# mickeyjoe666/PHFPFAC

Measured on AMD Instinct MI355X. Metric: input GB/s scanned, higher is better.
Workload: dtype u8

## Files before the change

### phfpfac_amd/csrc/pfac_hip.hip

```cpp
#include <hip/hip_runtime.h>
#include <hip/hip_ext.h>

#include <stdint.h>
#include <stdio.h>
#include <stdlib.h>
#include <string.h>

#include <algorithm>
#include <chrono>
#include <mutex>
#include <type_traits>
#include <string>
#include <vector>

#include "pfac.h"
#include "pfac_fold.h"

namespace {

constexpr int WAVE = 64;
constexpr int SUB = WAVE * 16;
constexpr int SUBS = 4;
constexpr int WTILE = SUB * SUBS;
constexpr int MSUBS = 2;
// ... 1753 lines not shown
__global__ void __launch_bounds__(COUNT_THREADS_MAX)
pfac_count_kernel(const void *rec, const unsigned long long *tix, unsigned long long n_items, unsigned long long cap, unsigned n_states,
                  unsigned bins, unsigned long long *counts, unsigned long long *res) {
    extern __shared__ __attribute__((aligned(16))) unsigned char smem[];
    unsigned *lds = reinterpret_cast<unsigned *>(smem);
    const unsigned words = DIRECT ? n_states : 2 * bins;
    for (unsigned i = threadIdx.x; i < words; i += blockDim.x) lds[i] = 0;
    __syncthreads();
    const int lane = threadIdx.x & (WAVE - 1);
    const unsigned long long wstride = (unsigned long long)gridDim.x * (blockDim.x >> 6);
    unsigned long long counted = 0;
    unsigned phase = 0;
    bool peel = false;
    for (unsigned long long t = (unsigned long long)blockIdx.x * (blockDim.x >> 6) + (threadIdx.x >> 6); t < n_items; t += wstride) {
        if (BYTES == 0) {
            const unsigned long long i = t * WAVE + lane, n = cap;
            unsigned st = 0;
            bool have = i < n;
            if (have) st = static_cast<const pfac_record *>(rec)[i].state;
            have = have && st < n_states;
            counted += have;
            count_chunk<DIRECT>(lds, bins, counts, have, st, lane, phase, peel);
        } else {
            const unsigned long long e = tix[t], lo = e & TIX_BASE_MASK;
            const unsigned cnt = (unsigned)(e >> TIX_CNT_SHIFT);
            for (unsigned i0 = 0; i0 < cnt; i0 += WAVE) {
                const unsigned i = i0 + (unsigned)lane;
                unsigned pos, st = 0;
                bool have = i < cnt && lo + i < cap;
                if (have) heap_record<(BYTES ? BYTES : 4)>(rec, lo + i, t, pos, st);
                have = have && st < n_states;
                counted += have;
                count_chunk<DIRECT>(lds, bins, counts, have, st, lane, phase, peel);
            }
        }
    }
    __syncthreads();
    for (unsigned i = threadIdx.x; i < (DIRECT ? n_states : bins); i += blockDim.x) {
        const unsigned c = DIRECT ? lds[i] : lds[2 * i + 1];
        const unsigned st = DIRECT ? i : lds[2 * i] - 1u;
        if (c) __hip_atomic_fetch_add(counts + st, (unsigned long long)c, __ATOMIC_RELAXED, __HIP_MEMORY_SCOPE_AGENT);
    }
    counted = wave_sum64(counted);
    if (lane == 0 && counted) __hip_atomic_fetch_add(res, counted, __ATOMIC_RELAXED, __HIP_MEMORY_SCOPE_AGENT);
}

__global__ void pfac_sel_check_kernel(const pfac_record *sel, unsigned long long n, unsigned n_states, unsigned long long *bad) {
    const unsigned long long stride = (unsigned long long)gridDim.x * blockDim.x;
    bool wrong = false;
    for (unsigned long long i = (unsigned long long)blockIdx.x * blockDim.x + threadIdx.x; i < n; i += stride) {
        const pfac_record r = sel[i];
        wrong = wrong || r.state >= n_states || (i + 1 < n && sel[i + 1].pos <= r.pos);
    }
    if (wrong) bad[0] = 1ull;
}

constexpr int XGROUP = 64;
__global__ void pfac_tix_group_sum_kernel(const unsigned long long *tix, unsigned long long n_tiles, unsigned long long *gsum, unsigned n_groups) {
    const int lane = threadIdx.x & (WAVE - 1);
    const unsigned g = blockIdx.x * (blockDim.x >> 6) + (threadIdx.x >> 6);
    if (g >= n_groups) return;
    const unsigned long long t = (unsigned long long)g * XGROUP + lane;
    const unsigned c = t < n_tiles ? (unsigned)(tix[t] >> TIX_CNT_SHIFT) : 0u;
    const unsigned long long sum = wave_sum64(c);
    if (lane == 0) gsum[g] = sum;
}
__global__ void pfac_scan_groups_kernel(unsigned long long *gsum, unsigned n_groups) {
    __shared__ unsigned long long part[1024];
    const unsigned per = (n_groups + 1023u) / 1024u;
    const unsigned lo = threadIdx.x * per, hi = lo + per < n_groups ? lo + per : n_groups;
    unsigned long long sum = 0;
    for (unsigned i = lo; i < hi; i++) sum += gsum[i];
    part[threadIdx.x] = sum;
    __syncthreads();
    if (threadIdx.x == 0) {
        unsigned long long acc = 0;
        for (int i = 0; i < 1024; i++) { const unsigned long long v = part[i]; part[i] = acc; acc += v; }
    }
    __syncthreads();
    unsigned long long acc = part[threadIdx.x];
    for (unsigned i = lo; i < hi; i++) { const unsigned long long v = gsum[i]; gsum[i] = acc; acc += v; }
    if (hi == n_groups && lo < hi) gsum[n_groups] = acc;
}
template <int BYTES>
__global__ void pfac_expand_kernel(const void *rec, const unsigned long long *tix, unsigned long long n_tiles,
                                   const unsigned long long *gpre, unsigned n_groups, unsigned long long cap,
                                   unsigned long long first, unsigned long long n, pfac_record *out) {
    const int lane = threadIdx.x & (WAVE - 1);
    const unsigned g = blockIdx.x * (blockDim.x >> 6) + (threadIdx.x >> 6);
    if (g >= n_groups) return;
    const unsigned long long t = (unsigned long long)g * XGROUP + lane;
    const unsigned long long e = t < n_tiles ? tix[t] : 0ull;
    const unsigned c = (unsigned)(e >> TIX_CNT_SHIFT);
    const unsigned long long lo = e & TIX_BASE_MASK;
    const unsigned long long off = gpre[g] + (wave_incl_scan(c) - c);
    const unsigned long long end = first + n;
    for (int j = 0; j < XGROUP; j++) {
        const unsigned tc = __shfl(c, j, WAVE);
        if (tc == 0) continue;
        const unsigned long long tlo = __shfl(lo, j, WAVE), toff = __shfl(off, j, WAVE);
        if (toff >= end || toff + tc <= first) continue;
        for (unsigned i = (unsigned)lane; i < tc; i += WAVE) {
            const unsigned long long k = toff + i;
            if (k < first || k >= end || tlo + i >= cap) continue;
            pfac_record o;
            heap_record<BYTES>(rec, tlo + i, (unsigned long long)g * XGROUP + j, o.pos, o.state);
            out[k - first] = o;
        }
    }
}


__device__ __forceinline__ unsigned long long doc_lower_bound(const unsigned long long *off, unsigned long long n, unsigned long long x) {
    unsigned long long lo = 0, hi = n;
    while (lo < hi) {
        const unsigned long long mid = (lo + hi) >> 1;
        if (off[mid] < x) lo = mid + 1;
        else hi = mid;
    }
    return lo;
}
__device__ __forceinline__ unsigned long long doc_of(const unsigned long long *off, unsigned long long lo, unsigned long long hi, unsigned long long pos) {
    while (lo < hi) {
        const unsigned long long mid = (lo + hi + 1) >> 1;
        if (off[mid] <= pos) lo = mid;
        else hi = mid - 1;
    }
    return lo;
}
__device__ __forceinline__ void tile_docs(const unsigned long long *off, unsigned long long n_docs, unsigned long long t,
                                          unsigned long long n_tiles, unsigned long long &ds, unsigned long long &de,
                                          unsigned long long &dlo, unsigned long long &dhi) {
    ds = doc_lower_bound(off, n_docs + 1, t * WTILE);
    de = t + 1 == n_tiles ? n_docs + 1 : doc_lower_bound(off, n_docs + 1, (t + 1) * WTILE);
    const unsigned long long top = n_docs - 1;
    dlo = ds ? ds - 1 : 0;
    dhi = de ? de - 1 : 0;
    if (dlo > top) dlo = top;
    if (dhi > top) dhi = top;
    if (dhi < dlo) dhi = dlo;
}

struct DocWin {
    unsigned long long dlo, dhi, woff;
    unsigned n, top;
    bool win;
};
__device__ __forceinline__ DocWin doc_window(const unsigned long long *off, unsigned long long dlo, unsigned long long dhi, int lane) {
    DocWin w;
    w.dlo = dlo;
    w.dhi = dhi;
    w.win = dhi - dlo + 2 <= (unsigned long long)WAVE;
    w.n = w.win ? (unsigned)(dhi - dlo + 1) : 0u;
    w.top = w.n > 1 ? 1u << (31 - __clz(w.n - 1)) : 0u;
    w.woff = w.win && (unsigned)lane <= w.n ? off[dlo + lane] : ~0ull;
    return w;
}
__device__ __forceinline__ void doc_lookup(const DocWin &w, const unsigned long long *off, bool have, unsigned pos,
                                           unsigned long long &d, unsigned long long &base, unsigned long long &end) {
    if (w.win) {
        unsigned k = 0;
        for (unsigned step = w.top; step; step >>= 1) {
            const unsigned cand = k + step;
            const unsigned long long v = __shfl(w.woff, cand < w.n ? cand : 0u, WAVE);
            if (cand < w.n && v <= pos) k = cand;
        }
        d = w.dlo + k;
        base = __shfl(w.woff, k, WAVE);
        end = __shfl(w.woff, k + 1, WAVE);
    } else {
        d = have ? doc_of(off, w.dlo, w.dhi, pos) : w.dlo;
        base = have ? off[d] : 0ull;
        end = have ? off[d + 1] : 0ull;
    }
}
__device__ __forceinline__ int final_len(const short *flen, int freg, bool fsmall, bool have, unsigned st) {
    if (fsmall) return __shfl(freg, (int)st, WAVE);
    return have ? (int)flen[st] : 0;
}
#define GRID_THREAD ((unsigned long long)blockIdx.x * blockDim.x + threadIdx.x)
// ... 1098 lines not shown
        const unsigned l = rp_segment(so, cnt + 1, pos);
        const unsigned long long gs = so[l], ge = GAPS ? gs + sgl[l] : gs;
        unsigned long long pe;
        if (GAPS && pos < ge) {
            pe = min(ge, e);
            rp_merge(acc, in, (long long)(ssrc[l] + o - gs), n_avail, (unsigned)(pos - o), (unsigned)(pe - o));
        } else if constexpr (!TEMPLATES) {
            pe = min(so[l + 1], e);
            rp_merge(acc, rep, (long long)sro[l] + (long long)(o - ge), rep_size, (unsigned)(pos - o), (unsigned)(pe - o));
        } else {
            const unsigned long long m0 = ge + ssp[l], m1 = m0 + sml[l];
            if (pos < m0) {
                pe = min(m0, e);
                rp_merge(acc, rep, (long long)sro[l] + (long long)(o - ge), rep_size, (unsigned)(pos - o), (unsigned)(pe - o));
            } else if (pos < m1) {
                pe = min(m1, e);
                rp_merge(acc, in, (long long)(ssrc[l] + (ge - gs)) + (long long)(o - m0), n_avail, (unsigned)(pos - o), (unsigned)(pe - o));
            } else {
                pe = min(so[l + 1], e);
                rp_merge(acc, rep, (long long)sro[l] + (long long)ssp[l] + (long long)(o - m1), rep_size, (unsigned)(pos - o), (unsigned)(pe - o));
            }
        }
        return pe;
    });
}

template <bool TEMPLATES, bool GAPS>
__global__ void __launch_bounds__(4 * WAVE)
pfac_rp_doc_delta_kernel(const pfac_record *sel, unsigned long long n, const short *flen, const unsigned *roff,
                         const unsigned long long *X, const unsigned long long *gpre, unsigned long long *D,
                         const unsigned *split) {
    const int lane = threadIdx.x & (WAVE - 1);
    const unsigned long long b = (unsigned long long)blockIdx.x * 4 + (threadIdx.x >> 6), k = b * RP_BLOCK + (unsigned)lane;
    if (b * RP_BLOCK >= n) return;
    unsigned long long dk = 0;
    if (k < n) {
        const pfac_record r = sel[k];
        if constexpr (!TEMPLATES && GAPS) {
            dk = (unsigned long long)((long long)(roff[r.state + 1] - roff[r.state]) - (long long)flen[r.state]);
        } else {
            bool quote = false;
            if constexpr (TEMPLATES) quote = split[r.state] != PFAC_TEMPLATE_PLAIN;
            const long long R = (long long)(roff[r.state + 1] - roff[r.state]), L = (long long)flen[r.state];
            dk = (unsigned long long)(R + (quote ? L : 0ll) - (GAPS ? L : 0ll));
        }
    }
    unsigned long long base = 0;
    if (b > 0) {
        if constexpr (GAPS) {
            const pfac_record r = sel[b * RP_BLOCK - 1];
            base = X[b] + gpre[b / RP_GROUP] - ((unsigned long long)r.pos + (unsigned long long)flen[r.state]);
        } else {
            base = X[b] + gpre[b / RP_GROUP];
        }
    }
    rp_block_offsets(base, dk, k, n, D);
}

__global__ void pfac_rp_doc_offsets_kernel(const unsigned long long *off, const unsigned long long *doc_first,
                                           unsigned long long n_docs, const unsigned long long *D, unsigned long long n,
                                           unsigned long long *out_off) {
    const unsigned long long stride = (unsigned long long)gridDim.x * blockDim.x;
    for (unsigned long long d = (unsigned long long)blockIdx.x * blockDim.x + threadIdx.x; d <= n_docs; d += stride) {
        const unsigned long long f = doc_first[d];
        out_off[d] = off[d] + (n ? D[f < n ? f : n] : 0ull);
    }
}

__device__ __forceinline__ unsigned ndigits32(unsigned v) {
    return 1u + (v >= 10u) + (v >= 100u) + (v >= 1000u) + (v >= 10000u) + (v >= 100000u) + (v >= 1000000u) + (v >= 10000000u) +
           (v >= 100000000u) + (v >= 1000000000u);
}
__device__ __forceinline__ unsigned ndigits64(unsigned long long v) {
    return v < 1000000000ull ? ndigits32((unsigned)v) : 9u + ndigits32((unsigned)(v / 1000000000ull));
}
__device__ __forceinline__ unsigned text_line_len(unsigned long long pos, unsigned id) {
    const unsigned dp = ndigits64(pos);
    return 12u + (dp < 4u ? 4u : dp) + 16u + ndigits32(id) + 1u;
}
constexpr int TEXT_LINE_MAX = 12 + 18 + 16 + 10 + 1;
constexpr int TEXT_IMG = 16 + WAVE * TEXT_LINE_MAX + 15;

template <int BYTES>
__global__ void pfac_text_size_kernel(const void *rec, const unsigned long long *tix, unsigned long long n_tiles, unsigned long long cap,
                                      unsigned long long base, const int *idmap, unsigned long long *gsum, unsigned n_groups) {
    const int lane = threadIdx.x & (WAVE - 1);
    const unsigned g = blockIdx.x * (blockDim.x >> 6) + (threadIdx.x >> 6);
    if (g >= n_groups) return;
    const unsigned long long t = (unsigned long long)g * XGROUP + lane;
    const unsigned long long e = t < n_tiles ? tix[t] : 0ull;
    const unsigned c = (unsigned)(e >> TIX_CNT_SHIFT);
    const unsigned long long lo = e & TIX_BASE_MASK;
    unsigned long long total = 0;
    for (int j = 0; j < XGROUP; j++) {
        const unsigned tc = __shfl(c, j, WAVE);
        if (tc == 0) continue;
        const unsigned long long tlo = __shfl(lo, j, WAVE);
        unsigned long long sum = 0;
        for (unsigned i = (unsigned)lane; i < tc && tlo + i < cap; i += WAVE) {
            unsigned pos, st;
            heap_record<BYTES>(rec, tlo + i, (unsigned long long)g * XGROUP + j, pos, st);
            sum += text_line_len(base + pos, (unsigned)idmap[st]);
        }
        total += sum;
    }
    total = wave_sum64(total);
    if (lane == 0) gsum[g] = total;
}

__device__ __forceinline__ void put_digits32(unsigned char *p, unsigned v, unsigned nd) {
    for (unsigned k = nd; k-- > 0;) { const unsigned q = v / 10u; p[k] = (unsigned char)('0' + (v - q * 10u)); v = q; }
}

template <int BYTES>
__global__ __launch_bounds__(256) void pfac_text_format_kernel(const void *rec, const unsigned long long *tix, unsigned long long n_tiles,
                                                               unsigned long long cap, unsigned long long base, const int *idmap,
                                                               const unsigned long long *gpre, unsigned n_groups, unsigned char *text) {
    __shared__ __attribute__((aligned(16))) unsigned char img_all[4][(TEXT_IMG + 15) / 16 * 16];
    const int lane = threadIdx.x & (WAVE - 1);
    unsigned char *img = img_all[threadIdx.x >> 6];
    const unsigned g = blockIdx.x * (blockDim.x >> 6) + (threadIdx.x >> 6);
    if (g >= n_groups) return;
    const unsigned long long t = (unsigned long long)g * XGROUP + lane;
    const unsigned long long e = t < n_tiles ? tix[t] : 0ull;
    const unsigned c = (unsigned)(e >> TIX_CNT_SHIFT);
    const unsigned long long lo = e & TIX_BASE_MASK;
    unsigned long long at = gpre[g];
    for (int j = 0; j < XGROUP; j++) {
        const unsigned tc = __shfl(c, j, WAVE);
        if (tc == 0) continue;
        const unsigned long long tlo = __shfl(lo, j, WAVE);
        for (unsigned c0 = 0; c0 < tc; c0 += WAVE) {
            const unsigned i = c0 + (unsigned)lane;
            const bool have = i < tc && tlo + i < cap;
            unsigned pos = 0, st = 0, id = 0, len = 0, dp = 0, di = 0;
            unsigned long long gp = 0;
            if (have) {
                heap_record<BYTES>(rec, tlo + i, (unsigned long long)g * XGROUP + j, pos, st);
                id = (unsigned)idmap[st];
                gp = base + pos;
                dp = ndigits64(gp);
                di = ndigits32(id);
                len = 12u + (dp < 4u ? 4u : dp) + 16u + di + 1u;
            }
            const unsigned incl = wave_incl_scan(len);
            const unsigned total = bcast_last(incl);
            const unsigned a0 = (unsigned)(at & 15ull);
            if (have) {
                unsigned char *p = img + a0 + (incl - len);
                const char *h = "At position ";
#pragma unroll
                for (int k = 0; k < 12; k++) p[k] = (unsigned char)h[k];
                p += 12;
                for (unsigned k = dp; k < 4u; k++) *p++ = ' ';
                if (gp < 1000000000ull) put_digits32(p, (unsigned)gp, dp);
                else {
                    const unsigned hi = (unsigned)(gp / 1000000000ull), lo9 = (unsigned)(gp - (unsigned long long)hi * 1000000000ull);
                    put_digits32(p, hi, dp - 9u);
                    put_digits32(p + (dp - 9u), lo9, 9u);
                }
                p += dp;
                const char *m = ", match pattern ";
#pragma unroll
                for (int k = 0; k < 16; k++) p[k] = (unsigned char)m[k];
                p += 16;
                put_digits32(p, id, di);
                p[di] = (unsigned char)'\n';
            }
            wave_lds_sync();
            unsigned char *dst = text + (at - a0);
            const unsigned end = a0 + total;
            const unsigned b_lo = a0 ? 16u : 0u, b_hi = end & ~15u;
            if (b_hi > b_lo) {
                for (unsigned o = b_lo + 16u * (unsigned)lane; o < b_hi; o += 16u * WAVE)
                    __builtin_nontemporal_store(*reinterpret_cast<const u32x4 *>(img + o), reinterpret_cast<u32x4 *>(dst + o));
                if (a0 && (unsigned)lane < 16u - a0) dst[a0 + lane] = img[a0 + lane];
                if ((unsigned)lane < end - b_hi) dst[b_hi + lane] = img[b_hi + lane];
            } else {
                if (a0 + (unsigned)lane < end) dst[a0 + lane] = img[a0 + lane];
            }
            wave_lds_sync();
            at += total;
        }
    }
}

__device__ __forceinline__ unsigned long long splitmix64(unsigned long long x) {
    x += 0x9E3779B97F4A7C15ull;
    x = (x ^ (x >> 30)) * 0xBF58476D1CE4E5B9ull;
    x = (x ^ (x >> 27)) * 0x94D049BB133111EBull;
    return x ^ (x >> 31);
}

__global__ void pfac_fill_random_kernel(unsigned long long *dst, unsigned long long n_words, unsigned long long seed) {
    const unsigned long long stride = (unsigned long long)gridDim.x * blockDim.x;
    for (unsigned long long i = (unsigned long long)blockIdx.x * blockDim.x + threadIdx.x; i < n_words; i += stride)
        dst[i] = splitmix64(seed + i);
}

__global__ void pfac_fill_tiled_kernel(unsigned char *dst, unsigned long long n, const unsigned char *pat,
                                       unsigned period, unsigned long long phase) {
    const unsigned long long stride = (unsigned long long)gridDim.x * blockDim.x * 16;
    for (unsigned long long i = ((unsigned long long)blockIdx.x * blockDim.x + threadIdx.x) * 16; i < n; i += stride) {
        unsigned k = (unsigned)((phase + i) % period);
        if (i + 16 <= n) {
            union { unsigned char b[16]; uint4 v; } u;
#pragma unroll
            for (int j = 0; j < 16; j++) { u.b[j] = pat[k]; k = k + 1 == period ? 0 : k + 1; }
            *reinterpret_cast<uint4 *>(dst + i) = u.v;
        } else {
            for (unsigned long long j = i; j < n; j++) { dst[j] = pat[k]; k = k + 1 == period ? 0 : k + 1; }
// ... 1710 lines not shown
    }
    if (n_tiles == 0) {
        if (ctx->event_timing) HIP_TRY(ctx, hipEventRecord(s.ev1, s.stream));
        __atomic_store_n(s.h_ctl + H_DONE, 1u, __ATOMIC_RELEASE);
    }
    return PFAC_OK;
}

int pfac_scan_finish(pfac_ctx *ctx, int slot, uint64_t *n_matches) {
    int rc = check_slot(ctx, slot);
    if (rc) return rc;
    Slot &s = ctx->slots[slot];
    if (!s.scanned) return fail(ctx, PFAC_E_STATE, "pfac_scan_finish without a scan");
    USE_DEVICE(ctx);
    rc = wait_scan(ctx, s);
    if (rc) return rc;
    if (s.last_tiles == 0 && s.h2d_issued) HIP_TRY(ctx, hipEventSynchronize(s.ev_h2d));
    s.pending = false;
    const uint64_t total = host_u64(s, H_MATCHES);
    s.last_total = total;
    s.last_used = host_u64(s, H_USED);
    if (n_matches) *n_matches = total;
#ifdef PFAC_TRACE_BUILD
    if (s.dbg.p && !ctx->plan.knobs.trace_file.empty()) {
        std::vector<unsigned long long> h(8 * 64 * 32);
        if (hipMemcpy(h.data(), s.dbg.p, h.size() * 8, hipMemcpyDeviceToHost) == hipSuccess) {
            if (FILE *f = fopen(ctx->plan.knobs.trace_file.c_str(), "wb")) { fwrite(h.data(), 8, h.size(), f); fclose(f); }
        }
    }
#endif
    if (s.h_ctl[2] != 0) {
        s.clean[0] = s.clean[1] = false;
        return fail(ctx, PFAC_E_INTERNAL, "scan kernel reported a timeout (flags " + std::to_string(s.h_ctl[2]) +
                                          ": 4 arrivals, 8 record base, 16 batch ring)");
    }
    if (ctx->plan.knobs.dense < 0 && ctx->plan.lay_d.stage_cap && s.last_tiles >= 64) {
        const uint64_t ovf = s.h_ctl[3];
        if (!ctx->dense && ovf * 4 > s.last_tiles) ctx->dense = true;
        else if (ctx->dense && ovf * 16 < s.last_tiles) ctx->dense = false;
    }
    if (ctx->plan.lag2_ok && ctx->plan.knobs.lag != 1 && ctx->plan.knobs.lag != 2 && s.last_tiles >= 64) {
        const uint64_t ovf2 = s.h_ctl[6];
        if (ctx->lag2 && ovf2 * 16 > s.last_tiles) ctx->lag2 = false;
        else if (!ctx->lag2 && ovf2 * 64 < s.last_tiles) ctx->lag2 = true;
    }
    if (s.last_used > s.last_cap)
        return fail(ctx, PFAC_E_OVERFLOW, "record array too small: " + std::to_string(total) + " matches need " +
                                              std::to_string(s.last_used) + " records of capacity (pfac_scan_capacity_hint)");
    return PFAC_OK;
}

int pfac_scan_elapsed_ms(pfac_ctx *ctx, int slot, float *ms) {
    int rc = check_slot(ctx, slot);
    if (rc) return rc;
    if (!ms) return fail(ctx, PFAC_E_ARG, "null argument");
    Slot &s = ctx->slots[slot];
    if (!s.scanned) return fail(ctx, PFAC_E_STATE, "no scan to time");
    USE_DEVICE(ctx);
    rc = wait_scan(ctx, s);
    if (rc) return rc;
    if (s.last_tiles == 0) *ms = 0.0f;
    else if (ctx->event_timing) {
        HIP_TRY(ctx, hipEventElapsedTime(ms, s.ev0, s.ev1));
        ctx->clk_diff_ms += *ms - (double)(host_u64(s, H_T1) - host_u64(s, H_T0)) * ctx->tick_ms;
        ctx->clk_n++;
    }
    else *ms = (float)((double)(host_u64(s, H_T1) - host_u64(s, H_T0)) * ctx->tick_ms);
    return PFAC_OK;
}

static int expand_records(pfac_ctx *ctx, Slot &s, const void *src, uint64_t first, uint64_t n, pfac_record *d_out) {
    if (s.pending) return fail(ctx, PFAC_E_STATE, "records requested before pfac_scan_finish");
    if (!in_window(first, n, s.last_total)) return fail(ctx, PFAC_E_ARG, "records [first, first + n) exceed the scan's match count");
    int rc = last_scan_usable(ctx, s, "", SCAN_FITS);
    if (rc) return rc;
    if (n == 0 || s.last_tiles == 0) return PFAC_OK;
    const unsigned n_groups = (unsigned)((s.last_tiles + XGROUP - 1) / XGROUP);
    rc = ensure_gsum(ctx, s, n_groups);
    if (rc) return rc;
    const unsigned gblocks = (n_groups + 3) / 4;
    hipLaunchKernelGGL(pfac_tix_group_sum_kernel, dim3(gblocks), dim3(256), 0, s.stream, s.tile_index.p,
                       (unsigned long long)s.last_tiles, s.gsum.p, n_groups);
    hipLaunchKernelGGL(pfac_scan_groups_kernel, dim3(1), dim3(1024), 0, s.stream, s.gsum.p, n_groups);
    auto ek = by_width(s.last_rec_bytes, [](auto w) { return pfac_expand_kernel<w()>; });
    hipLaunchKernelGGL(ek, dim3(gblocks), dim3(256), 0, s.stream, src, s.tile_index.p, (unsigned long long)s.last_tiles,
                       s.gsum.p, n_groups, (unsigned long long)s.last_cap, (unsigned long long)first, (unsigned long long)n, d_out);
    HIP_TRY(ctx, hipGetLastError());
    return PFAC_OK;
}

int pfac_scan_format(pfac_ctx *ctx, int slot, int *record_bytes, uint64_t *n_tiles, uint64_t *used) {
    int rc = check_slot(ctx, slot);
    if (rc) return rc;
    Slot &s = ctx->slots[slot];
    if (!s.scanned) return fail(ctx, PFAC_E_STATE, "no scan yet");
    if (record_bytes) *record_bytes = s.last_rec_bytes;
    if (n_tiles) *n_tiles = s.last_tiles;
    if (used) *used = s.last_used;
    return PFAC_OK;
}

int pfac_scan_capacity_hint(pfac_ctx *ctx, int slot, uint64_t *capacity) {
    int rc = check_slot(ctx, slot);
    if (rc) return rc;
    Slot &s = ctx->slots[slot];
    if (!s.scanned || !capacity) return fail(ctx, PFAC_E_STATE, "pfac_scan_capacity_hint: no finished scan");
    const uint64_t a = s.last_used + s.last_used / 8, b = s.last_total + s.last_total / 4;
    *capacity = (a > b ? a : b) + 65536;
    return PFAC_OK;
}

int pfac_records_expand(pfac_ctx *ctx, int slot, const void *d_records, uint64_t first, uint64_t n, pfac_record *d_out) {
    int rc = check_slot(ctx, slot);
    if (rc) return rc;
    Slot &s = ctx->slots[slot];
    const void *src = d_records ? d_records : s.records.p;
    if (!s.scanned) return fail(ctx, PFAC_E_STATE, "pfac_records_expand without a scan");
    if (!src || (!d_out && n) || ((uintptr_t)d_out & 7)) return fail(ctx, PFAC_E_ARG, "pfac_records_expand: bad buffer");
    USE_DEVICE(ctx);
    return expand_records(ctx, s, src, first, n, d_out);
}

int pfac_records_d2h(pfac_ctx *ctx, int slot, const void *d_records, pfac_record *host, uint64_t first, uint64_t n) {
    int rc = check_slot(ctx, slot);
    if (rc) return rc;
    Slot &s = ctx->slots[slot];
    const void *src = d_records ? d_records : s.records.p;
    if (n == 0) return PFAC_OK;
    if (!s.scanned) return fail(ctx, PFAC_E_STATE, "pfac_records_d2h without a scan");
    if (!src || !host) return fail(ctx, PFAC_E_ARG, "pfac_records_d2h: null buffer");
    USE_DEVICE(ctx);
    rc = s.wide.ensure(ctx, s.stream, n, n);
    if (rc) return rc;
    rc = expand_records(ctx, s, src, first, n, s.wide.p);
    if (rc) return rc;
    HIP_TRY(ctx, hipMemcpyAsync(host, s.wide.p, n * sizeof(pfac_record), hipMemcpyDeviceToHost, s.stream));
    return PFAC_OK;
}

int pfac_records_d2h_packed(pfac_ctx *ctx, int slot, const void *d_records, void *host_words, uint64_t n_words,
                            uint64_t *host_tile_index) {
    int rc = check_slot(ctx, slot);
    if (rc) return rc;
    Slot &s = ctx->slots[slot];
    const void *src = d_records ? d_records : s.records.p;
    if (!s.scanned || s.last_rec_bytes == 8) return fail(ctx, PFAC_E_STATE, "pfac_records_d2h_packed: the slot's last scan did not produce compact records");
    if (!src || (!host_words && n_words) || !host_tile_index) return fail(ctx, PFAC_E_ARG, "pfac_records_d2h_packed: null buffer");
    if (n_words > s.last_cap) return fail(ctx, PFAC_E_ARG, "pfac_records_d2h_packed: more words than the record array holds");
    USE_DEVICE(ctx);
    if (n_words) HIP_TRY(ctx, hipMemcpyAsync(host_words, src, n_words * (uint64_t)s.last_rec_bytes, hipMemcpyDeviceToHost, s.stream));
    if (s.last_tiles) HIP_TRY(ctx, hipMemcpyAsync(host_tile_index, s.tile_index.p, s.last_tiles * 8, hipMemcpyDeviceToHost, s.stream));
    return PFAC_OK;
}

int pfac_records_packed_device(pfac_ctx *ctx, int slot, const void *d_records, void *d_words_out, uint64_t n_words,
                               uint64_t *d_tile_index_out) {
    int rc = check_slot(ctx, slot);
    if (rc) return rc;
    Slot &s = ctx->slots[slot];
    const void *src = d_records ? d_records : s.records.p;
    if (!s.scanned || s.pending || s.last_rec_bytes == 8) return fail(ctx, PFAC_E_STATE, "pfac_records_packed_device: the slot's last finished scan did not produce compact records");
    rc = last_scan_usable(ctx, s, "", SCAN_FITS);
    if (rc) return rc;
    if (!d_tile_index_out || (d_words_out && !src)) return fail(ctx, PFAC_E_ARG, "pfac_records_packed_device: null buffer");
    if (n_words > s.last_cap) return fail(ctx, PFAC_E_ARG, "pfac_records_packed_device: more words than the record array holds");
    USE_DEVICE(ctx);
    if (d_words_out && n_words && d_words_out != src)
        HIP_TRY(ctx, hipMemcpyAsync(d_words_out, src, n_words * (uint64_t)s.last_rec_bytes, hipMemcpyDeviceToDevice, s.stream));
    if (s.last_tiles) HIP_TRY(ctx, hipMemcpyAsync(d_tile_index_out, s.tile_index.p, s.last_tiles * 8, hipMemcpyDeviceToDevice, s.stream));
    return PFAC_OK;
}

int pfac_emit_text_device(pfac_ctx *ctx, int slot, const void *d_records, uint64_t base, uint64_t *n_bytes) {
    int rc = check_slot(ctx, slot);
    if (rc) return rc;
    if (!n_bytes) return fail(ctx, PFAC_E_ARG, "null argument");
    *n_bytes = 0;
    if (!ctx->have_table) return fail(ctx, PFAC_E_STATE, "no table uploaded");
    Slot &s = ctx->slots[slot];
    const void *src = d_records ? d_records : s.records.p;
    rc = last_scan_usable(ctx, s, "pfac_emit_text_device", SCAN_FINISHED | SCAN_IDMAP | SCAN_FITS);
    if (rc) return rc;
    if (base + (1ull << 32) >= 1000000000000000000ull) return fail(ctx, PFAC_E_ARG, "pfac_emit_text_device: positions must stay below 10^18");
    s.text_bytes = 0;
    if (s.last_total == 0 || s.last_tiles == 0) return PFAC_OK;
    if (!src) return fail(ctx, PFAC_E_ARG, "null record buffer");
    USE_DEVICE(ctx);
    const unsigned n_groups = (unsigned)((s.last_tiles + XGROUP - 1) / XGROUP);
    rc = ensure_gsum(ctx, s, n_groups);
    if (rc) return rc;
    const unsigned gblocks = (n_groups + 3) / 4;
    auto sk = by_width(s.last_rec_bytes, [](auto w) { return pfac_text_size_kernel<w()>; });
    hipLaunchKernelGGL(sk, dim3(gblocks), dim3(256), 0, s.stream, src, s.tile_index.p, (unsigned long long)s.last_tiles,
                       (unsigned long long)s.last_cap, (unsigned long long)base, ctx->plan.d_idmap, s.gsum.p, n_groups);
    hipLaunchKernelGGL(pfac_scan_groups_kernel, dim3(1), dim3(1024), 0, s.stream, s.gsum.p, n_groups);
    HIP_TRY(ctx, hipGetLastError());
    unsigned long long total = 0;
    HIP_TRY(ctx, hipMemcpyAsync(&total, s.gsum.p + n_groups, 8, hipMemcpyDeviceToHost, s.stream));
    HIP_TRY(ctx, hipStreamSynchronize(s.stream));
    rc = s.text.ensure(ctx, s.stream, total + 32, total + total / 8 + 4096);
    if (rc) return rc;
    auto fk = by_width(s.last_rec_bytes, [](auto w) { return pfac_text_format_kernel<w()>; });
    hipLaunchKernelGGL(fk, dim3(gblocks), dim3(256), 0, s.stream, src, s.tile_index.p, (unsigned long long)s.last_tiles,
                       (unsigned long long)s.last_cap, (unsigned long long)base, ctx->plan.d_idmap, s.gsum.p, n_groups, s.text.p);
    HIP_TRY(ctx, hipGetLastError());
    s.text_bytes = total;
    *n_bytes = total;
    return PFAC_OK;
}

int pfac_text_d2h(pfac_ctx *ctx, int slot, void *host, uint64_t first, uint64_t n) {
    int rc = check_slot(ctx, slot);
    if (rc) return rc;
    Slot &s = ctx->slots[slot];
    if (!in_window(first, n, s.text_bytes)) return fail(ctx, PFAC_E_ARG, "pfac_text_d2h: range exceeds the text of the slot's last pfac_emit_text_device");
    if (n == 0) return PFAC_OK;
    if (!host) return fail(ctx, PFAC_E_ARG, "null buffer");
    USE_DEVICE(ctx);
    HIP_TRY(ctx, hipMemcpyAsync(host, s.text.p + first, n, hipMemcpyDeviceToHost, s.stream));
    return PFAC_OK;
}

void *pfac_slot_text(pfac_ctx *ctx, int slot) { return check_slot(ctx, slot) ? nullptr : ctx->slots[slot].text.p; }

int pfac_slot_sync(pfac_ctx *ctx, int slot) {
    int rc = check_slot(ctx, slot);
    if (rc) return rc;
    USE_DEVICE(ctx);
    HIP_TRY(ctx, hipStreamSynchronize(ctx->slots[slot].stream));
    if (ctx->slots[slot].h2d_issued) HIP_TRY(ctx, hipEventSynchronize(ctx->slots[slot].ev_h2d));
    return PFAC_OK;
}

int pfac_records_checksum(pfac_ctx *ctx, int slot, const void *d_records, uint64_t n, uint64_t base, uint64_t *checksum) {
    int rc = check_slot(ctx, slot);
    if (rc) return rc;
    if (!checksum) return fail(ctx, PFAC_E_ARG, "null argument");
    if (!ctx->have_table) return fail(ctx, PFAC_E_STATE, "no table uploaded");
    Slot &s = ctx->slots[slot];
    const void *src = d_records ? d_records : s.records.p;
    rc = n ? last_scan_usable(ctx, s, "pfac_records_checksum", SCAN_FINISHED | SCAN_IDMAP | SCAN_FITS) : PFAC_OK;
    if (rc) return rc;
    if (!src && n) return fail(ctx, PFAC_E_ARG, "null record buffer");
    USE_DEVICE(ctx);
    HIP_TRY(ctx, hipMemsetAsync(s.sum.p, 0, 16, s.stream));
    if (n && s.last_tiles) {
        auto ck = by_width(s.last_rec_bytes, [](auto w) { return pfac_checksum_kernel<w()>; });
        hipLaunchKernelGGL(ck, dim3(1024), dim3(256), 0, s.stream, src, s.tile_index.p, (unsigned long long)s.last_tiles,
                           (unsigned long long)s.last_cap, (unsigned long long)base, ctx->plan.d_idmap, s.sum.p);
        HIP_TRY(ctx, hipGetLastError());
    }
    HIP_TRY(ctx, hipMemcpyAsync(s.h_ctl + H_CHECKSUM, s.sum.p, 8, hipMemcpyDeviceToHost, s.stream));
    HIP_TRY(ctx, hipStreamSynchronize(s.stream));
    *checksum = host_u64(s, H_CHECKSUM);
    return PFAC_OK;
}

}

namespace {

using CountKernel = void (*)(const void *, const unsigned long long *, unsigned long long, unsigned long long, unsigned, unsigned,
                             unsigned long long *, unsigned long long *);

int count_run(pfac_ctx *ctx, Slot &s, const std::string &fn, const void *heap, bool is_sel, const pfac_record *sel, uint64_t n_sel,
              bool check_sel, uint64_t *d_counts, uint64_t n_states, uint32_t flags, uint64_t *n_counted) {
    if (flags > PFAC_COUNT_ACCUMULATE) return fail(ctx, PFAC_E_ARG, fn + ": flags must be 0 or PFAC_COUNT_ACCUMULATE");
    if (n_states != (uint64_t)ctx->plan.base.num_final)
        return fail(ctx, PFAC_E_ARG, fn + ": n_states must be num_final of the uploaded table (" + std::to_string(ctx->plan.base.num_final) + ")");
    if ((uintptr_t)d_counts & 7) return fail(ctx, PFAC_E_ARG, fn + ": d_counts must be 8-byte aligned");
    const bool own = d_counts == nullptr, acc = (flags & PFAC_COUNT_ACCUMULATE) != 0;
    if (own && acc && s.cnt.done && s.cnt_table != ctx->table_gen)
        return fail(ctx, PFAC_E_STATE, fn + ": the slot's counts belong to an earlier table; they cannot be added to");
    const uint64_t expect = is_sel ? n_sel : s.last_total;
    const uint64_t n_items = is_sel ? (n_sel + WAVE - 1) / WAVE : s.last_tiles;
    if (!(is_sel ? (const void *)sel : heap) && n_items) return fail(ctx, PFAC_E_ARG, "null record buffer");
    USE_DEVICE(ctx);
    int rc = ensure_gsum(ctx, s, 1);
    if (rc) return rc;
    unsigned long long *res = s.gsum.p;
    const unsigned ns = (unsigned)n_states;
    if (check_sel && n_sel) {
        HIP_TRY(ctx, hipMemsetAsync(res, 0, 16, s.stream));
        const unsigned blocks = (unsigned)std::min<uint64_t>((n_sel + 255) / 256, 1024);
        hipLaunchKernelGGL(pfac_sel_check_kernel, dim3(blocks), dim3(256), 0, s.stream, sel, (unsigned long long)n_sel, ns, res + 1);
        rc = pass_words(ctx, s, res + 1, 1, H_PASS1);
        if (rc) return rc;
// ... 1516 lines not shown
```

Baseline: 5335.

## Split each 64-tile group across several waves in expand and text kernels

The expand, text-size and text-format kernels now give each wave a unit of XUNIT tiles instead of a whole 64-tile group, multiplying the number of waves by XGROUP/XUNIT. The text-size kernel runs one block per group and writes per-unit byte offsets, so the format kernel can start each unit at the right text position. This targets poor parallelism and load imbalance when few groups exist or when match counts are skewed. In exchange each wave still loads the group's tile index and prefix-scans it, so that work is repeated, and an extra offset array is kept in the gsum buffer. Launch bounds and restrict qualifiers are also added.

```diff
diff --git a/phfpfac_amd/csrc/pfac_hip.hip b/phfpfac_amd/csrc/pfac_hip.hip
--- a/phfpfac_amd/csrc/pfac_hip.hip
+++ b/phfpfac_amd/csrc/pfac_hip.hip
@@ -1859,20 +1859,30 @@
     for (unsigned i = lo; i < hi; i++) { const unsigned long long v = gsum[i]; gsum[i] = acc; acc += v; }
     if (hi == n_groups && lo < hi) gsum[n_groups] = acc;
 }
+#ifndef PFAC_XUNIT
+#define PFAC_XUNIT 8
+#endif
+constexpr int XUNIT = PFAC_XUNIT;
+constexpr int XUNITS = XGROUP / XUNIT;
+static_assert(XUNIT >= 4 && XUNIT <= XGROUP && (XUNIT & (XUNIT - 1)) == 0, "PFAC_XUNIT: 4, 8, 16, 32 or 64");
+
 template <int BYTES>
-__global__ void pfac_expand_kernel(const void *rec, const unsigned long long *tix, unsigned long long n_tiles,
-                                   const unsigned long long *gpre, unsigned n_groups, unsigned long long cap,
-                                   unsigned long long first, unsigned long long n, pfac_record *out) {
+__global__ void __launch_bounds__(256, 8)
+pfac_expand_kernel(const void *__restrict__ rec, const unsigned long long *__restrict__ tix, unsigned long long n_tiles,
+                   const unsigned long long *__restrict__ gpre, unsigned n_units, unsigned long long cap,
+                   unsigned long long first, unsigned long long n, pfac_record *__restrict__ out) {
     const int lane = threadIdx.x & (WAVE - 1);
-    const unsigned g = blockIdx.x * (blockDim.x >> 6) + (threadIdx.x >> 6);
-    if (g >= n_groups) return;
+    const unsigned u = blockIdx.x * (blockDim.x >> 6) + (threadIdx.x >> 6);
+    if (u >= n_units) return;
+    const unsigned g = u / XUNITS;
+    const int j0 = (int)(u % XUNITS) * XUNIT;
     const unsigned long long t = (unsigned long long)g * XGROUP + lane;
     const unsigned long long e = t < n_tiles ? tix[t] : 0ull;
     const unsigned c = (unsigned)(e >> TIX_CNT_SHIFT);
     const unsigned long long lo = e & TIX_BASE_MASK;
     const unsigned long long off = gpre[g] + (wave_incl_scan(c) - c);
     const unsigned long long end = first + n;
-    for (int j = 0; j < XGROUP; j++) {
+    for (int j = j0; j < j0 + XUNIT; j++) {
         const unsigned tc = __shfl(c, j, WAVE);
         if (tc == 0) continue;
         const unsigned long long tlo = __shfl(lo, j, WAVE), toff = __shfl(off, j, WAVE);
@@ -3137,17 +3147,19 @@
 constexpr int TEXT_IMG = 16 + WAVE * TEXT_LINE_MAX + 15;
 
 template <int BYTES>
-__global__ void pfac_text_size_kernel(const void *rec, const unsigned long long *tix, unsigned long long n_tiles, unsigned long long cap,
-                                      unsigned long long base, const int *idmap, unsigned long long *gsum, unsigned n_groups) {
-    const int lane = threadIdx.x & (WAVE - 1);
-    const unsigned g = blockIdx.x * (blockDim.x >> 6) + (threadIdx.x >> 6);
-    if (g >= n_groups) return;
+__global__ void __launch_bounds__(XUNITS * WAVE, 8)
+pfac_text_size_kernel(const void *__restrict__ rec, const unsigned long long *__restrict__ tix, unsigned long long n_tiles,
+                      unsigned long long cap, unsigned long long base, const int *__restrict__ idmap,
+                      unsigned long long *__restrict__ gsum, unsigned long long *__restrict__ uoff) {
+    __shared__ unsigned long long unit_bytes[XUNITS];
+    const int lane = threadIdx.x & (WAVE - 1), w = threadIdx.x >> 6;
+    const unsigned g = blockIdx.x;
     const unsigned long long t = (unsigned long long)g * XGROUP + lane;
     const unsigned long long e = t < n_tiles ? tix[t] : 0ull;
     const unsigned c = (unsigned)(e >> TIX_CNT_SHIFT);
     const unsigned long long lo = e & TIX_BASE_MASK;
     unsigned long long total = 0;
-    for (int j = 0; j < XGROUP; j++) {
+    for (int j = w * XUNIT; j < (w + 1) * XUNIT; j++) {
         const unsigned tc = __shfl(c, j, WAVE);
         if (tc == 0) continue;
         const unsigned long long tlo = __shfl(lo, j, WAVE);
@@ -3160,7 +3172,14 @@
         total += sum;
     }
     total = wave_sum64(total);
-    if (lane == 0) gsum[g] = total;
+    if (lane == 0) unit_bytes[w] = total;
+    __syncthreads();
+    if (threadIdx.x < XUNITS) {
+        unsigned long long front = 0;
+        for (int k = 0; k < (int)threadIdx.x; k++) front += unit_bytes[k];
+        uoff[(unsigned long long)g * XUNITS + threadIdx.x] = front;
+        if (threadIdx.x == XUNITS - 1) gsum[g] = front + unit_bytes[XUNITS - 1];
+    }
 }
 
 __device__ __forceinline__ void put_digits32(unsigned char *p, unsigned v, unsigned nd) {
@@ -3168,20 +3187,24 @@
 }
 
 template <int BYTES>
-__global__ __launch_bounds__(256) void pfac_text_format_kernel(const void *rec, const unsigned long long *tix, unsigned long long n_tiles,
-                                                               unsigned long long cap, unsigned long long base, const int *idmap,
-                                                               const unsigned long long *gpre, unsigned n_groups, unsigned char *text) {
+__global__ void __launch_bounds__(256, 8)
+pfac_text_format_kernel(const void *__restrict__ rec, const unsigned long long *__restrict__ tix, unsigned long long n_tiles,
+                        unsigned long long cap, unsigned long long base, const int *__restrict__ idmap,
+                        const unsigned long long *__restrict__ gpre, const unsigned long long *__restrict__ uoff, unsigned n_units,
+                        unsigned char *__restrict__ text) {
     __shared__ __attribute__((aligned(16))) unsigned char img_all[4][(TEXT_IMG + 15) / 16 * 16];
     const int lane = threadIdx.x & (WAVE - 1);
     unsigned char *img = img_all[threadIdx.x >> 6];
-    const unsigned g = blockIdx.x * (blockDim.x >> 6) + (threadIdx.x >> 6);
-    if (g >= n_groups) return;
+    const unsigned u = blockIdx.x * (blockDim.x >> 6) + (threadIdx.x >> 6);
+    if (u >= n_units) return;
+    const unsigned g = u / XUNITS;
+    const int j0 = (int)(u % XUNITS) * XUNIT;
     const unsigned long long t = (unsigned long long)g * XGROUP + lane;
     const unsigned long long e = t < n_tiles ? tix[t] : 0ull;
     const unsigned c = (unsigned)(e >> TIX_CNT_SHIFT);
     const unsigned long long lo = e & TIX_BASE_MASK;
-    unsigned long long at = gpre[g];
-    for (int j = 0; j < XGROUP; j++) {
+    unsigned long long at = gpre[g] + uoff[u];
+    for (int j = j0; j < j0 + XUNIT; j++) {
         const unsigned tc = __shfl(c, j, WAVE);
         if (tc == 0) continue;
         const unsigned long long tlo = __shfl(lo, j, WAVE);
@@ -5058,9 +5081,10 @@
     hipLaunchKernelGGL(pfac_tix_group_sum_kernel, dim3(gblocks), dim3(256), 0, s.stream, s.tile_index.p,
                        (unsigned long long)s.last_tiles, s.gsum.p, n_groups);
     hipLaunchKernelGGL(pfac_scan_groups_kernel, dim3(1), dim3(1024), 0, s.stream, s.gsum.p, n_groups);
+    const unsigned n_units = n_groups * XUNITS;
     auto ek = by_width(s.last_rec_bytes, [](auto w) { return pfac_expand_kernel<w()>; });
-    hipLaunchKernelGGL(ek, dim3(gblocks), dim3(256), 0, s.stream, src, s.tile_index.p, (unsigned long long)s.last_tiles,
-                       s.gsum.p, n_groups, (unsigned long long)s.last_cap, (unsigned long long)first, (unsigned long long)n, d_out);
+    hipLaunchKernelGGL(ek, dim3((n_units + 3) / 4), dim3(256), 0, s.stream, src, s.tile_index.p, (unsigned long long)s.last_tiles,
+                       s.gsum.p, n_units, (unsigned long long)s.last_cap, (unsigned long long)first, (unsigned long long)n, d_out);
     HIP_TRY(ctx, hipGetLastError());
     return PFAC_OK;
 }
@@ -5163,12 +5187,13 @@
     if (!src) return fail(ctx, PFAC_E_ARG, "null record buffer");
     USE_DEVICE(ctx);
     const unsigned n_groups = (unsigned)((s.last_tiles + XGROUP - 1) / XGROUP);
-    rc = ensure_gsum(ctx, s, n_groups);
-    if (rc) return rc;
-    const unsigned gblocks = (n_groups + 3) / 4;
+    const unsigned n_units = n_groups * XUNITS;
+    rc = ensure_gsum(ctx, s, n_groups + 1 + n_units);
+    if (rc) return rc;
+    unsigned long long *uoff = s.gsum.p + n_groups + 1;
     auto sk = by_width(s.last_rec_bytes, [](auto w) { return pfac_text_size_kernel<w()>; });
-    hipLaunchKernelGGL(sk, dim3(gblocks), dim3(256), 0, s.stream, src, s.tile_index.p, (unsigned long long)s.last_tiles,
-                       (unsigned long long)s.last_cap, (unsigned long long)base, ctx->plan.d_idmap, s.gsum.p, n_groups);
+    hipLaunchKernelGGL(sk, dim3(n_groups), dim3(XUNITS * WAVE), 0, s.stream, src, s.tile_index.p, (unsigned long long)s.last_tiles,
+                       (unsigned long long)s.last_cap, (unsigned long long)base, ctx->plan.d_idmap, s.gsum.p, uoff);
     hipLaunchKernelGGL(pfac_scan_groups_kernel, dim3(1), dim3(1024), 0, s.stream, s.gsum.p, n_groups);
     HIP_TRY(ctx, hipGetLastError());
     unsigned long long total = 0;
@@ -5177,8 +5202,8 @@
     rc = s.text.ensure(ctx, s.stream, total + 32, total + total / 8 + 4096);
     if (rc) return rc;
     auto fk = by_width(s.last_rec_bytes, [](auto w) { return pfac_text_format_kernel<w()>; });
-    hipLaunchKernelGGL(fk, dim3(gblocks), dim3(256), 0, s.stream, src, s.tile_index.p, (unsigned long long)s.last_tiles,
-                       (unsigned long long)s.last_cap, (unsigned long long)base, ctx->plan.d_idmap, s.gsum.p, n_groups, s.text.p);
+    hipLaunchKernelGGL(fk, dim3((n_units + 3) / 4), dim3(256), 0, s.stream, src, s.tile_index.p, (unsigned long long)s.last_tiles,
+                       (unsigned long long)s.last_cap, (unsigned long long)base, ctx->plan.d_idmap, s.gsum.p, uoff, n_units, s.text.p);
     HIP_TRY(ctx, hipGetLastError());
     s.text_bytes = total;
     *n_bytes = total;
```

After: 5359, median of 5. Within noise of the previous version (+0.4%).
